# laboshinl/loam_velodyne

Hardware: AMD Instinct MI355X
Metric: sweeps/sec (64-ring, 1M-pt map): feature extraction + odometry + scan-to-map registration (higher is better)
Workload: dtype f32

## Files before the change

loam_velodyne_amd/csrc/dev_math.hpp:

```cpp
#pragma once
#include <hip/hip_runtime.h>
#include <cfloat>

namespace loamx {

struct Pose {
  float rx, ry, rz, tx, ty, tz;
  float srx, crx, sry, cry, srz, crz;
};

__host__ __device__ inline void pose_set_angles(Pose& p, float rx, float ry, float rz) {
  p.rx = rx; p.ry = ry; p.rz = rz;
  p.srx = (float)sin((double)rx); p.crx = (float)cos((double)rx);
  p.sry = (float)sin((double)ry); p.cry = (float)cos((double)ry);
  p.srz = (float)sin((double)rz); p.crz = (float)cos((double)rz);
}

__host__ __device__ inline void rot_x(float& y, float& z, float c, float s) {
  float y0 = y;
  y = c * y0 - s * z;
  z = s * y0 + c * z;
}
__host__ __device__ inline void rot_y(float& x, float& z, float c, float s) {
  float x0 = x;
// ... 183 lines not shown
#pragma unroll
      for (int r = k; r < M; r++) A[r][c] -= dot * v[r];
    }
    {
      float dot = 0.f;
#pragma unroll
      for (int r = k; r < M; r++) dot += v[r] * b[r];
      dot *= tau;
#pragma unroll
      for (int r = k; r < M; r++) b[r] -= dot * v[r];
    }
  }
  float y[N];
#pragma unroll
  for (int c = 0; c < N; c++) y[c] = 0.f;
#pragma unroll
  for (int k = N - 1; k >= 0; k--) {
    if (k < nonzero) {
      float s = b[k];
#pragma unroll
      for (int c = k + 1; c < N; c++)
        if (c < nonzero) s -= A[k][c] * y[c];
      y[k] = s / A[k][k];
    }
  }
#pragma unroll
  for (int c = 0; c < N; c++) x[c] = 0.f;
#pragma unroll
  for (int c = 0; c < N; c++)
#pragma unroll
    for (int j = 0; j < N; j++)
      if (c < nonzero && perm[c] == j) x[j] = y[c];
}

__device__ __forceinline__ void eig6_sym(const float* Ain, float* w, float* V, float* ws) {
  float* A = ws;
  float* Q = ws + 36;
  for (int r = 0; r < 6; r++)
    for (int c = 0; c <= r; c++) A[r * 6 + c] = A[c * 6 + r] = Ain[r * 6 + c];
  for (int r = 0; r < 6; r++)
    for (int c = 0; c < 6; c++) Q[r * 6 + c] = (r == c) ? 1.f : 0.f;
  for (int sweep = 0; sweep < 16; sweep++) {
    float off = 0.f, diag = 0.f;
    for (int r = 0; r < 6; r++) {
      diag += A[r * 6 + r] * A[r * 6 + r];
      for (int c = 0; c < r; c++) off += A[r * 6 + c] * A[r * 6 + c];
    }
    if (off <= 1e-20f * diag || off == 0.f) break;
    for (int p = 0; p < 5; p++)
      for (int q = p + 1; q < 6; q++) {
        float apq = A[p * 6 + q];
        if (apq == 0.f) continue;
        float theta = (A[q * 6 + q] - A[p * 6 + p]) / (2.f * apq);
        float t = (theta >= 0.f ? 1.f : -1.f) / (fabsf(theta) + sqrtf(theta * theta + 1.f));
        float c = 1.f / sqrtf(t * t + 1.f), s = t * c;
        for (int k = 0; k < 6; k++) {
          float akp = A[k * 6 + p], akq = A[k * 6 + q];
          A[k * 6 + p] = c * akp - s * akq;
          A[k * 6 + q] = s * akp + c * akq;
        }
        for (int k = 0; k < 6; k++) {
          float apk = A[p * 6 + k], aqk = A[q * 6 + k];
          A[p * 6 + k] = c * apk - s * aqk;
          A[q * 6 + k] = s * apk + c * aqk;
        }
        for (int k = 0; k < 6; k++) {
          float qkp = Q[k * 6 + p], qkq = Q[k * 6 + q];
          Q[k * 6 + p] = c * qkp - s * qkq;
          Q[k * 6 + q] = s * qkp + c * qkq;
        }
      }
  }
  int order[6];
#pragma unroll
  for (int k = 0; k < 6; k++) order[k] = k;
#pragma unroll
  for (int a_ = 1; a_ < 6; a_++) {
#pragma unroll
    for (int b_ = 5; b_ > 0; b_--) {
      if (b_ <= a_) {
        const float eb = A[order[b_] * 6 + order[b_]], ea = A[order[b_ - 1] * 6 + order[b_ - 1]];
        if (eb < ea) { int t = order[b_]; order[b_] = order[b_ - 1]; order[b_ - 1] = t; }
      }
    }
  }
  for (int k = 0; k < 6; k++) {
    w[k] = A[order[k] * 6 + order[k]];
    for (int r = 0; r < 6; r++) V[r * 6 + k] = Q[r * 6 + order[k]];
  }
}

__device__ __forceinline__ bool inverse6(const float* Ain, float* inv, float* ws) {
  float* A = ws;
  for (int r = 0; r < 6; r++)
    for (int c = 0; c < 6; c++) {
      A[r * 12 + c] = Ain[r * 6 + c];
      A[r * 12 + 6 + c] = (r == c) ? 1.f : 0.f;
    }
  for (int k = 0; k < 6; k++) {
    int piv = k;
    for (int r = k + 1; r < 6; r++)
      if (fabsf(A[r * 12 + k]) > fabsf(A[piv * 12 + k])) piv = r;
    if (A[piv * 12 + k] == 0.f) return false;
    if (piv != k)
      for (int c = 0; c < 12; c++) { float t = A[k * 12 + c]; A[k * 12 + c] = A[piv * 12 + c]; A[piv * 12 + c] = t; }
    float d = 1.f / A[k * 12 + k];
    for (int c = 0; c < 12; c++) A[k * 12 + c] *= d;
    for (int r = 0; r < 6; r++)
      if (r != k) {
        float f = A[r * 12 + k];
        if (f != 0.f)
          for (int c = 0; c < 12; c++) A[r * 12 + c] -= f * A[k * 12 + c];
      }
  }
  for (int r = 0; r < 6; r++)
    for (int c = 0; c < 6; c++) inv[r * 6 + c] = A[r * 12 + 6 + c];
  return true;
}

__device__ __forceinline__ bool certainly_not_degenerate(const float* AtA, float thr) {
  double L[6][6];
  const double shift = (double)thr * 1.001;
  double scale = 0.0;
#pragma unroll
  for (int i = 0; i < 6; i++) scale = fmax(scale, fabs((double)AtA[i * 6 + i]));
  const double tiny = 1e-6 * scale;
#pragma unroll
  for (int j = 0; j < 6; j++) {
    double dj = (double)AtA[j * 6 + j] - shift;
#pragma unroll
    for (int k = 0; k < 6; k++)
      if (k < j) dj -= L[j][k] * L[j][k];
    if (!(dj > tiny)) return false;
    const double lj = sqrt(dj);
    L[j][j] = lj;
#pragma unroll
    for (int i = 0; i < 6; i++)
      if (i > j) {
        double s = (double)AtA[i * 6 + j];
#pragma unroll
        for (int k = 0; k < 6; k++)
          if (k < j) s -= L[i][k] * L[j][k];
        L[i][j] = s / lj;
      }
  }
  return true;
}

__device__ __forceinline__ bool degeneracy_projector_full(const float* AtA, float thr, float* P, float* ws);
__device__ __forceinline__ bool degeneracy_projector(const float* AtA, float thr, float* P, float* ws) {
  if (certainly_not_degenerate(AtA, thr)) return false;
  return degeneracy_projector_full(AtA, thr, P, ws);
}
__device__ __forceinline__ bool degeneracy_projector_full(const float* AtA, float thr, float* P, float* ws) {
  float w[6];
  float* V = ws + 72;
  float* V2 = ws + 108;
  float* Vi = ws + 144;
  eig6_sym(AtA, w, V, ws);
  for (int k = 0; k < 36; k++) V2[k] = V[k];
  bool degenerate = false;
  {
    bool go = true;
#pragma unroll
    for (int i = 0; i < 6; i++) {
      if (go && w[i] < thr) {
        for (int j = 0; j < 6; j++) V2[i * 6 + j] = 0.f;
        degenerate = true;
      } else {
        go = false;
      }
    }
  }
  if (!inverse6(V, Vi, ws)) {
    for (int k = 0; k < 36; k++) P[k] = (k % 7 == 0) ? 1.f : 0.f;
    return degenerate;
  }
  for (int r = 0; r < 6; r++)
    for (int c = 0; c < 6; c++) {
      float s = 0.f;
      for (int k = 0; k < 6; k++) s += Vi[r * 6 + k] * V2[k * 6 + c];
      P[r * 6 + c] = s;
    }
  return degenerate;
}

__device__ __forceinline__ float lane_get(float x, int lane) { return __int_as_float(__builtin_amdgcn_readlane(__float_as_int(x), lane)); }

__device__ __forceinline__ float qr_solve6_lanes(const float* AtA, const float* AtB) {
  const int gl = (int)(threadIdx.x & 63);
  float a[6];
#pragma unroll
  for (int r = 0; r < 6; r++) a[r] = gl < 6 ? AtA[r * 6 + gl] : (gl == 6 ? AtB[r] : 0.f);
  int L[6] = {0, 1, 2, 3, 4, 5};
  bool pivoted = false;
  float s0 = 0.f;
#pragma unroll
  for (int r = 0; r < 6; r++) s0 += a[r] * a[r];
  const float nrm = gl < 6 ? sqrtf(s0) : 0.f;
  float maxnorm = lane_get(nrm, 0);
#pragma unroll
  for (int c = 1; c < 6; c++) {
    const float v = lane_get(nrm, c);
    maxnorm = v > maxnorm ? v : maxnorm;
  }
  const float thr_helper = (maxnorm * FLT_EPSILON) * (maxnorm * FLT_EPSILON) / 6.0f;
  int nonzero = 6;
#pragma unroll
  for (int k = 0; k < 6; k++) {
    float s = 0.f, tail = 0.f;
#pragma unroll
    for (int r = k; r < 6; r++) s += a[r] * a[r];
#pragma unroll
    for (int r = k + 1; r < 6; r++) tail += a[r] * a[r];
    const float c0 = a[k];
    float tau, beta, v[6];
    if (tail <= FLT_MIN) {
      tau = 0.f;
      beta = c0;
#pragma unroll
      for (int r = 0; r < 6; r++) v[r] = 0.f;
    } else {
      beta = sqrtf(c0 * c0 + tail);
      if (c0 >= 0.f) beta = -beta;
#pragma unroll
      for (int r = 0; r < 6; r++) v[r] = r > k ? a[r] / (c0 - beta) : 0.f;
      tau = (beta - c0) / beta;
    }
    v[k] = 1.f;
    int best = k;
    float bestn = lane_get(s, L[k]);
#pragma unroll
    for (int c = k + 1; c < 6; c++) {
      const float sc = lane_get(s, L[c]);
      if (sc > bestn) { bestn = sc; best = c; }
    }
    best = __builtin_amdgcn_readfirstlane(best);
    if (nonzero == 6 && bestn < thr_helper * float(6 - k)) nonzero = k;
    {
      int lb = L[k];
#pragma unroll
      for (int c = k + 1; c < 6; c++) lb = best == c ? L[c] : lb;
#pragma unroll
      for (int c = k + 1; c < 6; c++) L[c] = best == c ? L[k] : L[c];
      L[k] = __builtin_amdgcn_readfirstlane(lb);
    }
    const int pl = L[k];
    tau = lane_get(tau, pl);
    beta = lane_get(beta, pl);
#pragma unroll
    for (int r = k + 1; r < 6; r++) v[r] = lane_get(v[r], pl);
    if (gl == pl) {
      pivoted = true;
      a[k] = beta;
#pragma unroll
      for (int r = k + 1; r < 6; r++) a[r] = 0.f;
    } else if (gl <= 6 && !pivoted) {
      float dot = 0.f;
#pragma unroll
      for (int r = k; r < 6; r++) dot += v[r] * a[r];
      dot *= tau;
#pragma unroll
      for (int r = k; r < 6; r++) a[r] -= dot * v[r];
    }
  }
  float y = 0.f;
#pragma unroll
  for (int k = 5; k >= 0; k--) {
    float sacc = lane_get(a[k], 6);
#pragma unroll
    for (int c = k + 1; c < 6; c++) {
      const float term = lane_get(a[k] * y, L[c]);
      if (c < nonzero) sacc -= term;
    }
    const float diag = lane_get(a[k], L[k]);
    if (gl == L[k] && k < nonzero) y = sacc / diag;
  }
  return gl < 6 ? y : 0.f;
}
__device__ __forceinline__ void qr_solve6_coop(const float* AtA, const float* AtB, float* X) {
  const float y = qr_solve6_lanes(AtA, AtB);
  if ((threadIdx.x & 63) < 6) X[threadIdx.x & 63] = y;
}

__device__ __forceinline__ void xchg_store(double* p, double v) { __hip_atomic_store(p, v, __ATOMIC_RELAXED, __HIP_MEMORY_SCOPE_AGENT); }
__device__ __forceinline__ void xchg_stores_done() { asm volatile("s_waitcnt vmcnt(0)" ::: "memory"); }
__device__ __forceinline__ double xchg_load_nowait(const double* p) {
  double v;
  asm volatile("global_load_dwordx2 %0, %1, off sc1" : "=v"(v) : "v"(p) : "memory");
  return v;
}
typedef unsigned xrec_t __attribute__((ext_vector_type(4)));
__device__ __forceinline__ void xrec_store(xrec_t* p, double v, unsigned tag) {
  xrec_t r;
  r.x = tag; r.y = (unsigned)__double2loint(v); r.z = (unsigned)__double2hiint(v); r.w = tag;
  asm volatile("global_store_dwordx4 %0, %1, off sc1\n\ts_nop 1" ::"v"(p), "v"(r) : "memory");
}
__device__ __forceinline__ xrec_t xrec_load(const xrec_t* p) {
  xrec_t r;
  asm volatile("global_load_dwordx4 %0, %1, off sc1\n\ts_waitcnt vmcnt(0)" : "=v"(r) : "v"(p) : "memory");
  return r;
}
__device__ __forceinline__ double xrec_value(const xrec_t& r) { return __hiloint2double((int)r.z, (int)r.y); }
__device__ __forceinline__ void xchg_loads_done() { asm volatile("s_waitcnt vmcnt(0)" ::: "memory"); }
__device__ __forceinline__ void xchg_loaded(double& v) { asm volatile("" : "+v"(v)); }

}
```

loam_velodyne_amd/csrc/odometry.hip:

```cpp
#include "odometry.hpp"
#include "odom_schedule.hpp"
#include "pinned_copy.hpp"
#include <chrono>
#include <cstring>
#include <type_traits>

namespace loamx {

constexpr int OD_THREADS = 256;
constexpr int OD_TR_STRIDE = OD_THREADS + 2;
constexpr int OD_PART_STRIDE = 2 * (2 * 16 * LX_NSUM) + 16;
[[maybe_unused]] constexpr int OD_PART_TS = 2 * (2 * 16 * LX_NSUM);

__device__ inline void sincos_f(float a, float& s, float& c) { sincosf(a, &s, &c); }

__device__ inline void transform_to_start(const float* T, float scan_period, const float4 pi, float& x, float& y, float& z) {
  const float s = (1.f / scan_period) * (pi.w - (float)(int)pi.w);
  x = pi.x - s * T[3];
  y = pi.y - s * T[4];
  z = pi.z - s * T[5];
  float sx, cx, sy, cy, sz, cz;
  sincos_f(-s * T[0], sx, cx);
  sincos_f(-s * T[1], sy, cy);
  sincos_f(-s * T[2], sz, cz);
// ... 124 lines not shown
template <bool LOAD_FIRST, class F>
__device__ inline void block27_scan(const Block27& B, const float4* __restrict__ sorted, int lane, Block27First& first, F&& visit) {
  for (uint32_t c0 = (uint32_t)lane; c0 < B.total; c0 += 4 * 64) {
    const bool first_trip = c0 == (uint32_t)lane;
    uint32_t pos[4];
    float4 p[4];
#pragma unroll
    for (int u = 0; u < 4; u++) {
      const uint32_t cc = c0 + 64u * u;
      uint32_t o = B.O[8];
#pragma unroll
      for (int k = 7; k >= 0; k--) o = cc < B.E[k] ? B.O[k] : o;
      pos[u] = cc < B.total ? cc + o : B.O[0];
    }
    if (LOAD_FIRST || !first_trip) {
#pragma unroll
      for (int u = 0; u < 4; u++) p[u] = sorted[pos[u]];
      if (LOAD_FIRST && first_trip) {
#pragma unroll
        for (int u = 0; u < OD_BLK_CACHE; u++) first.p[u] = p[u];
      }
    } else {
#pragma unroll
      for (int u = OD_BLK_CACHE; u < 4; u++) p[u] = sorted[pos[u]];
#pragma unroll
      for (int u = 0; u < OD_BLK_CACHE; u++) p[u] = first.p[u];
    }
#pragma unroll
    for (int u = 0; u < 4; u++) visit(p[u], (c0 + 64u * u) < B.total);
  }
}
__device__ inline int nn1_block(const GridDesc& g, const Block27& B, const float4* __restrict__ sorted, const uint32_t* __restrict__ cell_start,
                                float qx, float qy, float qz, int lane, uint32_t& w_out, Block27First& first) {
  float lbest = 25.0f;
  uint32_t lw = 0xffffffffu;
  block27_scan<true>(B, sorted, lane, first, [&](const float4& p, bool valid) {
    const float dx = qx - p.x, dy2 = qy - p.y, dz2 = qz - p.z;
    const float d2 = dx * dx + dy2 * dy2 + dz2 * dz2;
    const uint32_t w = __float_as_uint(p.w);
    if (valid && (d2 < lbest || (d2 == lbest && lw != 0xffffffffu && (w & OD_IDX_MASK) < (lw & OD_IDX_MASK)))) { lbest = d2; lw = w; }
  });
  float d = lbest;
  int j = lw == 0xffffffffu ? -1 : (int)(lw & OD_IDX_MASK), o_ = lw == 0xffffffffu ? 0x7fffffff : (int)(lw & OD_IDX_MASK);
  int ring = (int)(lw >> 24);
  {
#pragma unroll
    for (int off = 32; off > 0; off >>= 1) {
      const float od = __shfl_xor(d, off, 64);
      const int oj = __shfl_xor(j, off, 64), oo = __shfl_xor(o_, off, 64), orr = __shfl_xor(ring, off, 64);
      if (od < d || (od == d && oo < o_)) { d = od; j = oj; o_ = oo; ring = orr; }
    }
  }
  const float h = 1.0f / g.inv_h;
  if (j >= 0 && d < 25.0f && d <= h * h) { w_out = ((uint32_t)ring << 24) | (uint32_t)j; return j; }
  const int id = nn1_shells(g, sorted, cell_start, qx, qy, qz, lane, 2, (j >= 0 && d < 25.0f) ? d : 25.0f, (j >= 0 && d < 25.0f) ? j : -1);
  w_out = id == j ? (((uint32_t)ring << 24) | (uint32_t)j) : (0xff000000u | (uint32_t)(id < 0 ? 0 : id));
  return id;
}

constexpr int OD_RF_N = 320;
#ifdef LOAMX_PROF_CORR
__device__ unsigned long long g_corr_ts[3][16];
#define OC_TS(k) do { if (blockIdx.y == 0 && lane == 0 && ts_slot >= 0) g_corr_ts[ts_slot][k] = wall_clock64(); } while (0)
#else
#define OC_TS(k) do { } while (0)
#endif
__global__ __launch_bounds__(256) OD_CORR_ATTR void k_odom_corr_grid(OdomProblem* __restrict__ probs, OdomParams P, uint32_t* __restrict__ patch_dst, uint4 patch) {
  if (patch_dst && blockIdx.x == 0 && blockIdx.y == 0 && threadIdx.x == 0) { patch_dst[0] = patch.x; patch_dst[1] = patch.y; patch_dst[2] = patch.z; }
  OdomProblem& pb = probs[blockIdx.y];
  if (pb.done) return;
  const int lane = threadIdx.x & 63, wid = threadIdx.x >> 6;
  const int nSharp = (int)pb.n_sharp, nFlat = (int)pb.n_flat;
  int f;
  {
    const int x = (int)(blockIdx.x % 8), j = (int)(blockIdx.x / 8);
    const int sS = (int)((long long)x * nSharp / 8), nS = (int)((long long)(x + 1) * nSharp / 8) - sS;
    const int sF = (int)((long long)x * nFlat / 8), nF = (int)((long long)(x + 1) * nFlat / 8) - sF;
    const int fl = 4 * j + wid;
    if (fl >= nS + nF) return;
    f = fl < nS ? sS + fl : nSharp + sF + (fl - nS);
  }
#ifdef LOAMX_PROF_CORR
  const int ts_slot = f == nSharp / 2 ? 0 : f == nSharp + nFlat / 2 ? 1 : f == nSharp + nFlat - 1 ? 2 : -1;
#endif
  OC_TS(0);
  float T[6];
#pragma unroll
  for (int k = 0; k < 6; k++) T[k] = pb.transform[k];
  const bool corner = f < nSharp;
  const float4 pi = corner ? pb.sharp[f] : pb.flat[f - nSharp];
  const uint32_t* __restrict__ tbl = corner ? pb.rf_corner : pb.rf_surf;
  const int e0 = max((int)pi.w - 8, 0);
  uint32_t tv = 0u, unordered_epoch = 0u;
  if (tbl) {
    if (e0 + lane < OD_RF_N - 1) tv = tbl[e0 + lane];
    unordered_epoch = tbl[OD_RF_N - 1];
  }
  float x, y, z;
  transform_to_start(T, P.scan_period, pi, x, y, z);
  const GridDescB gd = corner ? *pb.lc_desc : *pb.ls_desc;
  const float4* __restrict__ sorted = pb.sorted;
  const uint32_t* __restrict__ cell_start = pb.cell_table + gd.cell_base;
  OC_TS(1);
  Block27 B;
  block27_build(gd.g, cell_start, x, y, z, lane, B);
  OC_TS(2);
  uint32_t wbest = 0u;
  Block27First first;
  const int closest = nn1_block(gd.g, B, sorted, cell_start, x, y, z, lane, wbest, first);
  OC_TS(3);
  if (closest < 0) {
    if (lane == 0) { pb.ind[5 * f] = -1; pb.ind[5 * f + 1] = -1; pb.ind[5 * f + 2] = -1; }
    return;
  }
  const float4* last = corner ? pb.last_corner : pb.last_surf;
  const int nLast = corner ? (int)pb.n_last_corner : (int)pb.n_last_surf;
  const int nCur = corner ? nSharp : nFlat;
  const int bound = nCur < nLast ? nCur : nLast;
  const int cscan = (wbest >> 24) != 255u ? (int)(wbest >> 24) : (int)last[closest].w;
  float d2 = 25.f, d3 = 25.f;
  int j2 = -1, j3 = -1, o2 = 0x7fffffff, o3 = 0x7fffffff;
  auto better = [](float d, int order, float dbest, int obest) { return d < dbest || (d == dbest && obest != 0x7fffffff && order < obest); };

  bool via_block = false;
  if (tbl && unordered_epoch != pb.rf_epoch && cscan < 255 && B.total > 0u) {
    const unsigned long long valid = __ballot(e0 + lane < OD_RF_N - 1 && (tv >> 24) == pb.rf_epoch);
    auto first_from = [&](int ring) -> int {
      const int k = ring - e0;
      if (k >= 64) return nLast;
      const unsigned long long m = k <= 0 ? valid : (valid >> k) << k;
      if (!m) return nLast;
      const int w = (int)((uint32_t)__shfl((int)tv, __builtin_ctzll(m), 64) & OD_IDX_MASK);
      return w < nLast ? w : nLast;
    };
    if (cscan - 2 >= e0 || e0 == 0) {
      const int wlo = min(first_from(cscan - 2), closest);
      const int whi = closest + 1 < bound ? max(min(bound, first_from(cscan + 3)), closest + 1) : closest + 1;
      const unsigned walk = (unsigned)(closest - wlo) + (unsigned)(whi - (closest + 1));
      via_block = walk > B.total + 128u;
    }
  }
  OC_TS(4);
  if (via_block) {
    block27_scan<false>(B, sorted, lane, first, [&](const float4& p, bool ok) {
      const uint32_t w = __float_as_uint(p.w);
      const int j = (int)(w & OD_IDX_MASK), ring = (int)(w >> 24);
      const float d = sqd(p, x, y, z);
      if (ok && j > closest && j < bound && ring <= cscan + 2) {
        const int order = j - (closest + 1);
        if (corner) {
          if (ring > cscan && better(d, order, d2, o2)) { d2 = d; j2 = j; o2 = order; }
        } else {
          if (ring <= cscan) { if (better(d, order, d2, o2)) { d2 = d; j2 = j; o2 = order; } }
          else { if (better(d, order, d3, o3)) { d3 = d; j3 = j; o3 = order; } }
        }
      } else if (ok && j < closest && ring >= cscan - 2) {
        const int order = 0x40000000 + (closest - 1 - j);
        if (corner) {
          if (ring < cscan && better(d, order, d2, o2)) { d2 = d; j2 = j; o2 = order; }
        } else {
          if (ring >= cscan) { if (better(d, order, d2, o2)) { d2 = d; j2 = j; o2 = order; } }
          else { if (better(d, order, d3, o3)) { d3 = d; j3 = j; o3 = order; } }
        }
      }
    });
    wave_argmin(d2, j2, o2);
    if (!corner) wave_argmin(d3, j3, o3);
    const float h = 1.0f / gd.g.inv_h, h2 = h * h;
    via_block = d2 < h2 && (corner || d3 < h2);
    if (!via_block) { d2 = d3 = 25.f; j2 = j3 = -1; o2 = o3 = 0x7fffffff; }
  }
  OC_TS(5);
  if (!via_block) {
    int baseF = closest + 1, baseB = closest - 1;
    bool stopF = baseF >= bound, stopB = baseB < 0;
    while (!stopF || !stopB) {
      float4 qf[4], qb[4];
      if (!stopF) {
#pragma unroll
        for (int u = 0; u < 4; u++) {
          const int j = baseF + 64 * u + lane;
          qf[u] = j < bound ? last[j] : make_float4(0.f, 0.f, 0.f, 0.f);
        }
      }
      if (!stopB) {
#pragma unroll
        for (int u = 0; u < 4; u++) {
          const int j = baseB - 64 * u - lane;
          qb[u] = j >= 0 ? last[j] : make_float4(0.f, 0.f, 0.f, 0.f);
        }
      }
      if (!stopF) {
        bool stop = false;
#pragma unroll
        for (int u = 0; u < 4; u++) {
          if (stop) continue;
          const int j = baseF + 64 * u + lane;
          const bool in = j < bound;
          const int ring = (int)qf[u].w;
          const bool brk = in && ((double)ring > (double)cscan + 2.5);
          const unsigned long long mb = __ballot(brk);
          const int fb = mb ? __builtin_ctzll(mb) : 64;
          if (in && lane < fb) {
            const float d = sqd(qf[u], x, y, z);
            const int order = j - (closest + 1);
            if (corner) {
              if (ring > cscan && better(d, order, d2, o2)) { d2 = d; j2 = j; o2 = order; }
            } else {
              if (ring <= cscan) { if (better(d, order, d2, o2)) { d2 = d; j2 = j; o2 = order; } }
              else { if (better(d, order, d3, o3)) { d3 = d; j3 = j; o3 = order; } }
            }
          }
          if (mb) stop = true;
        }
        baseF += 256;
        stopF = stop || baseF >= bound;
      }
      if (!stopB) {
        bool stop = false;
#pragma unroll
        for (int u = 0; u < 4; u++) {
          if (stop) continue;
          const int j = baseB - 64 * u - lane;
          const bool in = j >= 0;
          const int ring = (int)qb[u].w;
          const bool brk = in && ((double)ring < (double)cscan - 2.5);
          const unsigned long long mb = __ballot(brk);
          const int fb = mb ? __builtin_ctzll(mb) : 64;
          if (in && lane < fb) {
            const float d = sqd(qb[u], x, y, z);
            const int order = 0x40000000 + (closest - 1 - j);
            if (corner) {
              if (ring < cscan && better(d, order, d2, o2)) { d2 = d; j2 = j; o2 = order; }
            } else {
              if (ring >= cscan) { if (better(d, order, d2, o2)) { d2 = d; j2 = j; o2 = order; } }
              else { if (better(d, order, d3, o3)) { d3 = d; j3 = j; o3 = order; } }
            }
          }
          if (mb) stop = true;
        }
        baseB -= 256;
        stopB = stop || baseB < 0;
      }
    }
    wave_argmin(d2, j2, o2);
    if (!corner) wave_argmin(d3, j3, o3);
  }
  OC_TS(6);
  if (lane == 0) {
    pb.ind[5 * f] = closest;
    pb.ind[5 * f + 1] = j2;
    pb.ind[5 * f + 2] = corner ? -1 : j3;
  }
#ifdef LOAMX_PROF_CORR
  if (blockIdx.y == 0 && lane == 0 && ts_slot >= 0) {
    g_corr_ts[ts_slot][7] = wall_clock64();
    g_corr_ts[ts_slot][8] = (unsigned long long)B.total; g_corr_ts[ts_slot][9] = (unsigned long long)via_block;
    g_corr_ts[ts_slot][10] = (unsigned long long)closest; g_corr_ts[ts_slot][11] = (unsigned long long)cscan;
  }
#endif
}

#ifdef LOAMX_PROF_LM
#define LM_TS(k) do { if (blockIdx.x == 0 && blockIdx.y == 0 && tid == 0 && iter == it_begin + 1) pb.part[OD_PART_TS + (k)] = (double)wall_clock64(); } while (0)
#else
#define LM_TS(k) do { } while (0)
#endif
#ifndef OD_LM_WAVES
#define OD_LM_WAVES 3
#endif
#ifndef OD_LM_WAVES_MIN
#define OD_LM_WAVES_MIN 3
#endif
#define OD_LM_ATTR __attribute__((amdgpu_waves_per_eu(OD_LM_WAVES_MIN, OD_LM_WAVES)))
#pragma clang diagnostic push
#pragma clang diagnostic ignored "-Wpass-failed"
template <int OD_FPT>
__global__ __launch_bounds__(OD_THREADS) OD_LM_ATTR void k_odom_lm(OdomProblem* __restrict__ probs, OdomParams P, int iter0, int n_iters) {
  OdomProblem& pb = probs[blockIdx.y];
  if (pb.done) return;
  const unsigned NB = gridDim.x;
  const int tid = threadIdx.x;
  const int nSharp = (int)pb.n_sharp, nFlat = (int)pb.n_flat, nFeat = nSharp + nFlat;
  __shared__ float T[6];
  __shared__ float trig[6];
  __shared__ double red[8][LX_NSUM];
  using TrT = typename std::conditional<OD_FPT == 1, float, double>::type;
  __shared__ TrT tr[LX_NSUM * OD_TR_STRIDE];
  __shared__ int sh_done, sh_degen, sh_abort;
  __shared__ float matP[36];
  __shared__ float ws[216];
  __shared__ double parts[16 * LX_NSUM];
  __shared__ float AtA[36], AtB[6];
  if (tid < 6) {
    T[tid] = pb.transform[tid];
    const double ang = (double)pb.transform[tid >> 1];
    trig[tid] = (float)((tid & 1) ? cos(ang) : sin(ang));
  }
  const unsigned xtag = pb.xchg_epoch << 8;
  if (tid == 0) { sh_done = 0; sh_abort = 0; sh_degen = pb.stats.degenerate; }
  if (tid < 36) matP[tid] = pb.matP[tid];
  __syncthreads();

  float4 fpo[OD_FPT], ft1[OD_FPT], ft2[OD_FPT], ft3[OD_FPT];
  bool fvalid[OD_FPT], fcorner[OD_FPT];
#pragma unroll
  for (int u = 0; u < OD_FPT; u++) {
    const int f = (u * (int)NB + (int)blockIdx.x) * OD_THREADS + tid;
    fvalid[u] = false;
    fcorner[u] = f < nSharp;
    fpo[u] = ft1[u] = ft2[u] = ft3[u] = make_float4(0.f, 0.f, 0.f, 0.f);
    if (f < nFeat) {
      const int i1 = pb.ind[5 * f], i2 = pb.ind[5 * f + 1], i3 = pb.ind[5 * f + 2];
      if (fcorner[u] ? (i2 >= 0) : (i2 >= 0 && i3 >= 0)) {
        fvalid[u] = true;
        fpo[u] = fcorner[u] ? pb.sharp[f] : pb.flat[f - nSharp];
        const float4* last = fcorner[u] ? pb.last_corner : pb.last_surf;
        ft1[u] = last[i1];
        ft2[u] = last[i2];
        if (!fcorner[u]) ft3[u] = last[i3];
      }
    }
  }

  const int it_begin = iter0, it_end = iter0 + n_iters;
  for (int iter = it_begin; iter < it_end; iter++) {
    LM_TS(0);
    LM_TS(1);
    double v[OD_FPT == 1 ? 1 : LX_NSUM];
    float a1[6] = {0.f, 0.f, 0.f, 0.f, 0.f, 0.f}, bb1 = 0.f;
    bool sel1 = false;
#pragma unroll
    for (int k = 0; k < (OD_FPT == 1 ? 1 : LX_NSUM); k++) v[k] = 0.0;
#pragma unroll
    for (int u = 0; u < OD_FPT; u++) {
      if (!fvalid[u]) continue;
      const bool corner = fcorner[u];
      const float4 po = fpo[u];
      float cx = 0.f, cy = 0.f, cz = 0.f, ci = 0.f;
      bool sel = false;
      {
        float x0, y0, z0;
        transform_to_start(T, P.scan_period, po, x0, y0, z0);
        if (corner) {
          const float4 t1 = ft1[u], t2 = ft2[u];
          const float x1 = t1.x, y1 = t1.y, z1 = t1.z, x2 = t2.x, y2 = t2.y, z2 = t2.z;
          const float a012 = sqrtf(((x0 - x1) * (y0 - y2) - (x0 - x2) * (y0 - y1)) * ((x0 - x1) * (y0 - y2) - (x0 - x2) * (y0 - y1)) +
                                   ((x0 - x1) * (z0 - z2) - (x0 - x2) * (z0 - z1)) * ((x0 - x1) * (z0 - z2) - (x0 - x2) * (z0 - z1)) +
                                   ((y0 - y1) * (z0 - z2) - (y0 - y2) * (z0 - z1)) * ((y0 - y1) * (z0 - z2) - (y0 - y2) * (z0 - z1)));
          const float l12 = sqrtf((x1 - x2) * (x1 - x2) + (y1 - y2) * (y1 - y2) + (z1 - z2) * (z1 - z2));
          const float la = ((y1 - y2) * ((x0 - x1) * (y0 - y2) - (x0 - x2) * (y0 - y1)) +
                            (z1 - z2) * ((x0 - x1) * (z0 - z2) - (x0 - x2) * (z0 - z1))) / a012 / l12;
          const float lb = -((x1 - x2) * ((x0 - x1) * (y0 - y2) - (x0 - x2) * (y0 - y1)) -
                             (z1 - z2) * ((y0 - y1) * (z0 - z2) - (y0 - y2) * (z0 - z1))) / a012 / l12;
          const float lc = -((x1 - x2) * ((x0 - x1) * (z0 - z2) - (x0 - x2) * (z0 - z1)) +
                             (y1 - y2) * ((y0 - y1) * (z0 - z2) - (y0 - y2) * (z0 - z1))) / a012 / l12;
          const float ld2 = a012 / l12;
          float s = 1;
          if (iter >= 5) s = 1 - 1.8f * fabsf(ld2);
          cx = s * la; cy = s * lb; cz = s * lc; ci = s * ld2;
          sel = ((double)s > 0.1) && (ld2 != 0);
        } else {
          const float4 t1 = ft1[u], t2 = ft2[u], t3 = ft3[u];
          float pa = (t2.y - t1.y) * (t3.z - t1.z) - (t3.y - t1.y) * (t2.z - t1.z);
          float pbb = (t2.z - t1.z) * (t3.x - t1.x) - (t3.z - t1.z) * (t2.x - t1.x);
          float pc = (t2.x - t1.x) * (t3.y - t1.y) - (t3.x - t1.x) * (t2.y - t1.y);
          float pd = -(pa * t1.x + pbb * t1.y + pc * t1.z);
          const float ps = sqrtf(pa * pa + pbb * pbb + pc * pc);
          pa /= ps; pbb /= ps; pc /= ps; pd /= ps;
          const float pd2 = pa * x0 + pbb * y0 + pc * z0 + pd;
          float s = 1;
          if (iter >= 5) s = 1 - 1.8f * fabsf(pd2) / sqrtf(sqrtf(x0 * x0 + y0 * y0 + z0 * z0));
          cx = s * pa; cy = s * pbb; cz = s * pc; ci = s * pd2;
          sel = ((double)s > 0.1) && (pd2 != 0);
        }
      }
      if (sel) {
        const float srx = trig[0], crx = trig[1], sry = trig[2], cry = trig[3], srz = trig[4], crz = trig[5];
        const float tx = T[3], ty = T[4], tz = T[5];
        const float px = po.x, py = po.y, pz = po.z;
        float a[6];
        a[0] = (-crx * sry * srz * px + crx * crz * sry * py + srx * sry * pz + tx * crx * sry * srz - ty * crx * crz * sry - tz * srx * sry) * cx +
               (srx * srz * px - crz * srx * py + crx * pz + ty * crz * srx - tz * crx - tx * srx * srz) * cy +
               (crx * cry * srz * px - crx * cry * crz * py - cry * srx * pz + tz * cry * srx + ty * crx * cry * crz - tx * crx * cry * srz) * cz;
        a[1] = ((-crz * sry - cry * srx * srz) * px + (cry * crz * srx - sry * srz) * py - crx * cry * pz + tx * (crz * sry + cry * srx * srz) +
                ty * (sry * srz - cry * crz * srx) + tz * crx * cry) * cx +
               ((cry * crz - srx * sry * srz) * px + (cry * srz + crz * srx * sry) * py - crx * sry * pz + tz * crx * sry -
                ty * (cry * srz + crz * srx * sry) - tx * (cry * crz - srx * sry * srz)) * cz;
        a[2] = ((-cry * srz - crz * srx * sry) * px + (cry * crz - srx * sry * srz) * py + tx * (cry * srz + crz * srx * sry) -
                ty * (cry * crz - srx * sry * srz)) * cx +
               (-crx * crz * px - crx * srz * py + ty * crx * srz + tx * crx * crz) * cy +
               ((cry * crz * srx - sry * srz) * px + (crz * sry + cry * srx * srz) * py + tx * (sry * srz - cry * crz * srx) -
                ty * (crz * sry + cry * srx * srz)) * cz;
        a[3] = -(cry * crz - srx * sry * srz) * cx + crx * srz * cy - (crz * sry + cry * srx * srz) * cz;
        a[4] = -(cry * srz + crz * srx * sry) * cx - crx * crz * cy - (sry * srz - cry * crz * srx) * cz;
        a[5] = crx * sry * cx - srx * cy - crx * cry * cz;
        const float bb = (float)(-0.05 * (double)ci);
        if (OD_FPT == 1) {
#pragma unroll
          for (int i = 0; i < 6; i++) a1[i] = a[i];
          bb1 = bb;
          sel1 = true;
        } else {
          int k = 0;
#pragma unroll
          for (int i = 0; i < 6; i++)
#pragma unroll
            for (int j = i; j < 6; j++) v[k++] += (double)(a[i] * a[j]);
#pragma unroll
          for (int i = 0; i < 6; i++) v[k++] += (double)(a[i] * bb);
          v[k] += 1.0;
        }
      }
    }
    LM_TS(2);
    if (OD_FPT == 1) {
      int k = 0;
#pragma unroll
      for (int i = 0; i < 6; i++)
#pragma unroll
        for (int j = i; j < 6; j++) tr[(k++) * OD_TR_STRIDE + tid] = (TrT)(a1[i] * a1[j]);
#pragma unroll
      for (int i = 0; i < 6; i++) tr[(k++) * OD_TR_STRIDE + tid] = (TrT)(a1[i] * bb1);
      tr[k * OD_TR_STRIDE + tid] = (TrT)(sel1 ? 1.f : 0.f);
    } else {
#pragma unroll
      for (int t = 0; t < LX_NSUM; t++) tr[t * OD_TR_STRIDE + tid] = (TrT)v[OD_FPT == 1 ? 0 : t];
    }
    __syncthreads();
    if (tid < 8 * LX_NSUM) {
      const int c = tid % LX_NSUM, g = tid / LX_NSUM;
      const TrT* col = tr + c * OD_TR_STRIDE + g;
      double x = 0.0;
#pragma unroll 8
      for (int j = 0; j < OD_THREADS / 8; j++) x += (double)col[8 * j];
      red[g][c] = x;
    }
    __syncthreads();
    LM_TS(3);
    double xs = 0.0;
    if (tid < LX_NSUM) {
#pragma unroll
      for (int w = 0; w < 8; w++) xs += red[w][tid];
      if (NB > 1) {
        xrec_store(reinterpret_cast<xrec_t*>(pb.part) + (((unsigned)iter & 1u) * 16u + blockIdx.x) * LX_NSUM + tid, xs, xtag | (unsigned)(iter + 1));
      }
    }
    if (NB > 1) {
      LM_TS(4);
      {
        const unsigned want = xtag | (unsigned)(iter + 1);
        const xrec_t* rec = reinterpret_cast<const xrec_t*>(pb.part) + ((unsigned)iter & 1u) * 16u * LX_NSUM;
        const unsigned long long t_in = wall_clock64();
        for (unsigned e = tid; e < NB * LX_NSUM; e += OD_THREADS) {
          unsigned spins = 0;
          xrec_t r = xrec_load(rec + e);
          while (r.x != want || r.w != want) {
            __builtin_amdgcn_s_sleep(1);
            if ((++spins & 1023u) == 0u && wall_clock64() - t_in > 200000000ull) { sh_abort = 1; break; }
            r = xrec_load(rec + e);
          }
          parts[e] = xrec_value(r);
        }
      }
      __syncthreads();
      if (sh_abort) {
        if (tid == 0) {
          pb.done = 1;
          if (pb.err_word) __hip_atomic_store(pb.err_word, 1u, __ATOMIC_RELAXED, __HIP_MEMORY_SCOPE_SYSTEM);
          if (pb.host_mirror) pb.host_mirror->done = -1;
        }
        return;
      }
      LM_TS(5);
    }
    if (tid < 64) {
      if (NB > 1 && tid < LX_NSUM) {
        xs = 0.0;
        for (unsigned b = 0; b < NB; b++) xs += parts[b * LX_NSUM + tid];
      }
      if (tid < 21) {
        int i = 0, rem = tid;
        while (rem >= 6 - i) { rem -= 6 - i; i++; }
        const int j = i + rem;
        AtA[i * 6 + j] = AtA[j * 6 + i] = (float)xs;
      } else if (tid < 27) {
        AtB[tid - 21] = (float)xs;
      }
      const int sel = (int)__hiloint2double(__builtin_amdgcn_readlane(__double2hiint(xs), 27), __builtin_amdgcn_readlane(__double2loint(xs), 27));
      __builtin_amdgcn_fence(__ATOMIC_SEQ_CST, "wavefront");
      LM_TS(7);
      float xl = 0.f;
      int done_now = 0;
      if (sel >= 10) {
        xl = qr_solve6_lanes(AtA, AtB);
        LM_TS(8);
        if (iter == 0) {
          if (tid == 0) sh_degen = degeneracy_projector(AtA, 10.f, matP, ws) ? 1 : 0;
          __builtin_amdgcn_fence(__ATOMIC_SEQ_CST, "wavefront");
          if (blockIdx.x == 0 && tid < 36) pb.matP[tid] = matP[tid];
        }
        const int degen = sh_degen;
        if (degen) {
          const int r = tid < 6 ? tid : 5;
          float acc = 0.f;
#pragma unroll
          for (int c = 0; c < 6; c++) acc += matP[r * 6 + c] * lane_get(xl, c);
          xl = acc;
        }
        float x6[6];
#pragma unroll
        for (int k = 0; k < 6; k++) x6[k] = lane_get(xl, k);
        const float d0 = (float)(x6[0] * 180.0 / M_PI), d1 = (float)(x6[1] * 180.0 / M_PI), d2 = (float)(x6[2] * 180.0 / M_PI);
        const float deltaR = (float)sqrt((double)d0 * d0 + (double)d1 * d1 + (double)d2 * d2);
        const float t0 = x6[3] * 100, t1 = x6[4] * 100, t2 = x6[5] * 100;
        const float deltaT = (float)sqrt((double)t0 * t0 + (double)t1 * t1 + (double)t2 * t2);
        done_now = (deltaR < P.delta_r_abort && deltaT < P.delta_t_abort) ? 1 : 0;
      }
      float tl = T[tid < 6 ? tid : 5];
      if (sel >= 10) {
        float nv = tl + xl;
        if (!isfinite(nv)) nv = 0.f;
        tl = nv;
      }
      const float a0 = lane_get(tl, 0), a1 = lane_get(tl, 1), a2 = lane_get(tl, 2);
      const double ang = (double)((tid >> 1) == 0 ? a0 : ((tid >> 1) == 1 ? a1 : a2));
      const float tg = (float)((tid & 1) ? cos(ang) : sin(ang));
      if (tid < 6) { T[tid] = tl; trig[tid] = tg; }
      if (tid == 0 && done_now) sh_done = 1;
      if (blockIdx.x == 0) {
        const bool final_now = done_now || iter == it_end - 1;
        if (tid < 6) pb.transform[tid] = tl;
        if (tid == 0) {
          pb.stats.iterations = iter + 1;
          pb.stats.sel = sel;
          if (iter == 0 && sel >= 10) pb.stats.degenerate = sh_degen;
          if (done_now) pb.done = 1;
        }
        if (final_now) {
          ToEndParams& Pe = *pb.te_out;
          if (tid < 6) {
            Pe.T[tid] = tl;
            if (tid & 1) Pe.cT[tid >> 1] = tg; else Pe.sT[tid >> 1] = tg;
          }
          if (pb.host_mirror) {
            OdomProblem* hm = pb.host_mirror;
            if (tid < 6) hm->transform[tid] = tl;
            if (tid == 0) {
              OdomStats stt;
              stt.iterations = iter + 1; stt.sel = sel; stt.frame = pb.stats.frame; stt.degenerate = sh_degen;
              hm->stats = stt;
              hm->done = done_now;
            }
          }
        }
      }
      LM_TS(9);
    }
    __syncthreads();
    if (sh_done) break;
  }
}

#pragma clang diagnostic pop

__device__ inline float4 to_end_point(float4 p, const ToEndParams& P) {
  const float s = (1.f / P.scan_period) * (p.w - (float)(int)p.w);
  float x = p.x - s * P.T[3], y = p.y - s * P.T[4], z = p.z - s * P.T[5];
  float sx, cx, sy, cy, sz, cz;
  sincos_f(-s * P.T[0], sx, cx);
  sincos_f(-s * P.T[1], sy, cy);
  sincos_f(-s * P.T[2], sz, cz);
  rot_z(x, y, cz, sz); rot_x(y, z, cx, sx); rot_y(x, z, cy, sy);
  rot_y(x, z, P.cT[1], P.sT[1]); rot_x(y, z, P.cT[0], P.sT[0]); rot_z(x, y, P.cT[2], P.sT[2]);
  x += P.T[3] - P.shift[0];
  y += P.T[4] - P.shift[1];
  z += P.T[5] - P.shift[2];
  rot_z(x, y, P.c_start[2], P.s_start[2]); rot_x(y, z, P.c_start[0], P.s_start[0]); rot_y(x, z, P.c_start[1], P.s_start[1]);
  rot_y(x, z, P.c_end[1], -P.s_end[1]); rot_x(y, z, P.c_end[0], -P.s_end[0]); rot_z(x, y, P.c_end[2], -P.s_end[2]);
  return make_float4(x, y, z, (float)(int)p.w);
}
__global__ __launch_bounds__(256) void k_transform_to_end_copy(float4* __restrict__ dst, const float4* __restrict__ src, uint32_t n, ToEndParams P) {
  const uint32_t i = blockIdx.x * blockDim.x + threadIdx.x;
  if (i >= n) return;
  dst[i] = to_end_point(src[i], P);
}
__global__ __launch_bounds__(256) void k_transform_to_end(float4* __restrict__ pts, uint32_t n, ToEndParams P) {
  const uint32_t i = blockIdx.x * blockDim.x + threadIdx.x;
  if (i >= n) return;
  pts[i] = to_end_point(pts[i], P);
}
__global__ void k_te_patch(const OdomProblem* __restrict__ probs, uint32_t na, ToEndParams* __restrict__ te) {
  const uint32_t a = blockIdx.x * blockDim.x + threadIdx.x;
  if (a >= na) return;
  const OdomProblem& pb = probs[a];
  ToEndParams& P = te[pb.stream_id];
  for (int k = 0; k < 6; k++) P.T[k] = pb.transform[k];
  for (int k = 0; k < 3; k++) {
    P.sT[k] = (float)sin((double)pb.transform[k]);
    P.cT[k] = (float)cos((double)pb.transform[k]);
  }
}

__global__ __launch_bounds__(256) void k_transform_to_end_batch(float4* __restrict__ pts, uint32_t n, const uint32_t* __restrict__ off,
                                                                uint32_t K, uint32_t ns, const ToEndParams* __restrict__ params,
                                                                const float4* __restrict__ src_c, const float4* __restrict__ src_s,
                                                                uint32_t n_corner_all, uint32_t* __restrict__ bounds,
                                                                uint32_t* __restrict__ ring_first, uint32_t rf_epoch) {
  const uint32_t i = blockIdx.x * blockDim.x + threadIdx.x;
  const bool active = i < n;
  uint32_t lo = 0;
  float4 q = make_float4(0.f, 0.f, 0.f, 0.f);
  if (active) {
    uint32_t hi = K;
    while (hi - lo > 1) {
      const uint32_t mid = (lo + hi) >> 1;
      if (off[mid] <= i) lo = mid; else hi = mid;
    }
    const ToEndParams P = params[lo % ns];
    if (src_c) {
      const float4 p = i < n_corner_all ? src_c[i] : src_s[i - n_corner_all];
      q = P.enabled ? to_end_point(p, P) : p;
      pts[i] = q;
    } else {
      q = pts[i];
      if (P.enabled) { q = to_end_point(q, P); pts[i] = q; }
    }
  }
  if (ring_first) {
    const int ring = (int)q.w;
    int prev = __shfl_up(ring, 1, 64);
    const uint32_t plo = (uint32_t)__shfl_up((int)lo, 1, 64);
    const bool first_in_cloud = active && i == off[lo];
    if (active && !first_in_cloud && (threadIdx.x & 63) == 0) {
      const uint32_t ip = i - 1;
      prev = (int)(src_c ? (ip < n_corner_all ? src_c[ip] : src_s[ip - n_corner_all]) : pts[ip]).w;
    } else if (active && plo != lo) {
      prev = -1;
    }
    if (active && ring >= 0 && ring < OD_RF_N - 1 && (first_in_cloud || prev != ring))
      ring_first[(size_t)lo * OD_RF_N + ring] = (rf_epoch << 24) | ((i - off[lo]) & OD_IDX_MASK);
    if (active && (ring < 0 || ring >= 255 || (i - off[lo]) > OD_IDX_MASK || (!first_in_cloud && prev > ring)))
      ring_first[(size_t)lo * OD_RF_N + OD_RF_N - 1] = rf_epoch;
  }
  if (bounds) cloud_bounds_update(bounds, active, lo, q.x, q.y, q.z);
}

__global__ __launch_bounds__(256) void k_to_end_gather(float4* __restrict__ dst, uint32_t n, const uint32_t* __restrict__ off, uint32_t K,
                                                       const float4* const* __restrict__ src, const uint32_t* __restrict__ sid,
                                                       const ToEndParams* __restrict__ params) {
  const uint32_t i = blockIdx.x * blockDim.x + threadIdx.x;
  if (i >= n) return;
  uint32_t lo = 0, hi = K;
  while (hi - lo > 1) {
    const uint32_t mid = (lo + hi) >> 1;
    if (off[mid] <= i) lo = mid; else hi = mid;
  }
  dst[i] = to_end_point(src[lo][i - off[lo]], params[sid[lo]]);
}

OdometryBatch::OdometryBatch(int device, uint32_t n_streams, hipStream_t shared_stream) : device_(device) {
  select_device(device);
  LX_REQUIRE(n_streams >= 1 && n_streams <= 1024, "n_streams must be in [1, 1024]");
  if (shared_stream) {
    st_ = shared_stream;
  } else {
    st_ = create_stream(env_priority("LOAMX_PRIO_ODOM", +1), 0, 0);
    own_stream_ = true;
  }
  for (uint32_t s = 0; s < n_streams; s++) streams_.push_back(new OdomStream());
  index_.cell_size = 2.1f;
  if (const char* e = diag_env("LOAMX_ODOM_CELL")) { const float v = (float)atof(e); if (v >= 0.25f && v <= 16.f) index_.cell_size = v; }
  index_.pack_ring = true;
  index_.init(st_);
  h_mirror_.reserve(n_streams);
  h_err_.reserve(16);
  rf_.reserve((size_t)2 * n_streams * OD_RF_N);
  LX_HIP(hipMemsetAsync(rf_.p, 0, sizeof(uint32_t) * 2 * n_streams * OD_RF_N, st_));
  memset(h_err_.p, 0, 16 * sizeof(uint32_t));
  part_.reserve((size_t)n_streams * OD_PART_STRIDE);
  LX_HIP(hipMemset(part_.p, 0, sizeof(double) * part_.cap));
  {
    auto up256 = [](size_t b) { return (b + 255) & ~(size_t)255; };
    const size_t o_te = up256(sizeof(OdomProblem) * n_streams), o_off = o_te + up256(sizeof(ToEndParams) * n_streams);
    up_bytes_ = o_off + up256(sizeof(uint32_t) * (2 * (size_t)n_streams + 2));
    up_dev_.reserve(up_bytes_);
    up_host_.reserve(up_bytes_);
    memset(up_host_.p, 0, up_bytes_);
    prob_.p = (OdomProblem*)up_dev_.p; h_prob_.p = (OdomProblem*)up_host_.p;
    te_.p = (ToEndParams*)(up_dev_.p + o_te); h_te_.p = (ToEndParams*)(up_host_.p + o_te);
    d_cur_off_.p = (uint32_t*)(up_dev_.p + o_off); h_off_pin_.p = (uint32_t*)(up_host_.p + o_off);
  }
  h_cur_off_.assign(2 * n_streams + 1, 0);
  h_last_off_.assign(2 * n_streams + 1, 0);
}

OdometryBatch::~OdometryBatch() {
  if (ev_tail_) (void)hipEventDestroy(ev_tail_);
  if (ev_up_) (void)hipEventDestroy(ev_up_);
  if (ev_pose_) (void)hipEventDestroy(ev_pose_);
  for (auto* p : streams_) delete p;
  for (auto& c : lt_) for (auto& e : c.ev) if (e) (void)hipEventDestroy(e);
  if (own_stream_ && st_) (void)hipStreamDestroy(st_);
}

void OdometryBatch::lt_resolve_() {
  for (auto& c : lt_) {
    if (!c.pending || !c.pairs) continue;
    if (hipEventQuery(c.ev[3 * (c.pairs - 1) + 2]) != hipSuccess) { (void)hipGetLastError(); continue; }
    for (int k = 0; k < c.pairs; k++) {
      float a = 0.f, b = 0.f;
      if (hipEventElapsedTime(&a, c.ev[3 * k], c.ev[3 * k + 1]) != hipSuccess || hipEventElapsedTime(&b, c.ev[3 * k + 1], c.ev[3 * k + 2]) != hipSuccess) { (void)hipGetLastError(); continue; }
      if (c.iters[k] > 0) {
        lt_tot_.corr_ms += a; lt_tot_.corr_launches++; lt_tot_.corr_features += c.feats[k];
        lt_tot_.lm_ms += b; lt_tot_.lm_launches++; lt_tot_.lm_iterations += (uint64_t)c.iters[k]; lt_tot_.lm_bytes += c.bytes[k];
      } else {
        lt_tot_.corr_noop_ms += a; lt_tot_.corr_noop_launches++;
        lt_tot_.lm_noop_ms += b; lt_tot_.lm_noop_launches++;
      }
    }
    c.pending = false;
  }
}
OdometryBatch::LaunchTotals OdometryBatch::launch_totals() {
  std::lock_guard<std::mutex> lk(lt_mu_);
  lt_resolve_();
  return lt_tot_;
}

void odom_set_imu(OdomStream& S, const float* t);
ToEndParams odom_to_end_params(const OdomStream& S, float scan_period, bool enabled);
void odom_integrate_pose(OdomStream& S);

void OdometryBatch::update_imu(uint32_t s, const float* t) { odom_set_imu(*streams_[s], t); }

ToEndParams OdometryBatch::to_end_params(uint32_t s, bool enabled) const { return odom_to_end_params(*streams_[s], params.scan_period, enabled); }

void OdometryBatch::to_end_device(uint32_t s, float4* pts, uint32_t n) {
  if (!n) return;
  hipLaunchKernelGGL(k_transform_to_end, dim3((n + 255) / 256), dim3(256), 0, st_, pts, n, to_end_params(s, true));
}

void odom_integrate_pose(OdomStream& S) {
  HAngle rx, ry, rz;
  accumulate_rotation(S.transform_sum.rot_x, S.transform_sum.rot_y, S.transform_sum.rot_z, -S.transform.rot_x,
                      HAngle((float)(-S.transform.rot_y.r * 1.05)), -S.transform.rot_z, rx, ry, rz);
  HVec3 v{S.transform.pos.x - S.imu_shift.x, S.transform.pos.y - S.imu_shift.y, (float)(S.transform.pos.z * 1.05 - S.imu_shift.z)};
  h_rot_zxy(v, rz, rx, ry);
  HVec3 trans{S.transform_sum.pos.x - v.x, S.transform_sum.pos.y - v.y, S.transform_sum.pos.z - v.z};
  plugin_imu_rotation(rx, ry, rz, S.imu_pitch_start, S.imu_yaw_start, S.imu_roll_start, S.imu_pitch_end, S.imu_yaw_end,
                      S.imu_roll_end, rx, ry, rz);
  S.transform_sum.rot_x = rx; S.transform_sum.rot_y = ry; S.transform_sum.rot_z = rz;
  S.transform_sum.pos = trans;
}
void odom_set_imu(OdomStream& S, const float* t) {
  S.imu_pitch_start = HAngle(t[0]); S.imu_yaw_start = HAngle(t[1]); S.imu_roll_start = HAngle(t[2]);
  S.imu_pitch_end = HAngle(t[3]); S.imu_yaw_end = HAngle(t[4]); S.imu_roll_end = HAngle(t[5]);
  S.imu_shift = {t[6], t[7], t[8]};
  S.imu_velo = {t[9], t[10], t[11]};
}
ToEndParams odom_to_end_params(const OdomStream& S, float scan_period, bool enabled) {
  ToEndParams P;
  S.transform.get(P.T);
  const HAngle* ta[3] = {&S.transform.rot_x, &S.transform.rot_y, &S.transform.rot_z};
  const HAngle* sa[3] = {&S.imu_pitch_start, &S.imu_yaw_start, &S.imu_roll_start};
// ... 475 lines not shown
```

Baseline: 16250.

## Precompute per-feature line/plane constants and batch cross-block exchange loads in one wavefront

Each feature's plane coefficients (surface) and line length (corner) are now computed once before the LM iteration loop and kept in registers, so later iterations no longer recompute them. The cross-block partial-sum exchange now uses only the first 64 threads. They issue up to eight dwordx4 loads back to back with a single wait, then spin only on records that were not yet ready. This is meant to cut per-iteration latency on the grid-wide reduction, the serial bottleneck of the iterative solver. It holds 7 floats per feature slot in registers and assumes NB*LX_NSUM fits in 512 records (8 x 64).

```diff
diff --git a/loam_velodyne_amd/csrc/dev_math.hpp b/loam_velodyne_amd/csrc/dev_math.hpp
--- a/loam_velodyne_amd/csrc/dev_math.hpp
+++ b/loam_velodyne_amd/csrc/dev_math.hpp
@@ -509,6 +509,12 @@
   return r;
 }
 __device__ __forceinline__ double xrec_value(const xrec_t& r) { return __hiloint2double((int)r.z, (int)r.y); }
+__device__ __forceinline__ xrec_t xrec_load_nowait(const xrec_t* p) {
+  xrec_t r;
+  asm volatile("global_load_dwordx4 %0, %1, off sc1" : "=v"(r) : "v"(p) : "memory");
+  return r;
+}
+__device__ __forceinline__ void xrec_loaded(xrec_t& r) { asm volatile("" : "+v"(r)); }
 __device__ __forceinline__ void xchg_loads_done() { asm volatile("s_waitcnt vmcnt(0)" ::: "memory"); }
 __device__ __forceinline__ void xchg_loaded(double& v) { asm volatile("" : "+v"(v)); }
 
diff --git a/loam_velodyne_amd/csrc/odometry.hip b/loam_velodyne_amd/csrc/odometry.hip
--- a/loam_velodyne_amd/csrc/odometry.hip
+++ b/loam_velodyne_amd/csrc/odometry.hip
@@ -450,23 +450,38 @@
   if (tid < 36) matP[tid] = pb.matP[tid];
   __syncthreads();
 
-  float4 fpo[OD_FPT], ft1[OD_FPT], ft2[OD_FPT], ft3[OD_FPT];
+  float4 fpo[OD_FPT];
+  float fk[OD_FPT][7];
   bool fvalid[OD_FPT], fcorner[OD_FPT];
 #pragma unroll
   for (int u = 0; u < OD_FPT; u++) {
     const int f = (u * (int)NB + (int)blockIdx.x) * OD_THREADS + tid;
     fvalid[u] = false;
     fcorner[u] = f < nSharp;
-    fpo[u] = ft1[u] = ft2[u] = ft3[u] = make_float4(0.f, 0.f, 0.f, 0.f);
+    fpo[u] = make_float4(0.f, 0.f, 0.f, 0.f);
+#pragma unroll
+    for (int k = 0; k < 7; k++) fk[u][k] = 0.f;
     if (f < nFeat) {
       const int i1 = pb.ind[5 * f], i2 = pb.ind[5 * f + 1], i3 = pb.ind[5 * f + 2];
       if (fcorner[u] ? (i2 >= 0) : (i2 >= 0 && i3 >= 0)) {
         fvalid[u] = true;
         fpo[u] = fcorner[u] ? pb.sharp[f] : pb.flat[f - nSharp];
         const float4* last = fcorner[u] ? pb.last_corner : pb.last_surf;
-        ft1[u] = last[i1];
-        ft2[u] = last[i2];
-        if (!fcorner[u]) ft3[u] = last[i3];
+        const float4 t1 = last[i1], t2 = last[i2];
+        if (fcorner[u]) {
+          const float x1 = t1.x, y1 = t1.y, z1 = t1.z, x2 = t2.x, y2 = t2.y, z2 = t2.z;
+          const float l12 = sqrtf((x1 - x2) * (x1 - x2) + (y1 - y2) * (y1 - y2) + (z1 - z2) * (z1 - z2));
+          fk[u][0] = x1; fk[u][1] = y1; fk[u][2] = z1; fk[u][3] = x2; fk[u][4] = y2; fk[u][5] = z2; fk[u][6] = l12;
+        } else {
+          const float4 t3 = last[i3];
+          float pa = (t2.y - t1.y) * (t3.z - t1.z) - (t3.y - t1.y) * (t2.z - t1.z);
+          float pbb = (t2.z - t1.z) * (t3.x - t1.x) - (t3.z - t1.z) * (t2.x - t1.x);
+          float pc = (t2.x - t1.x) * (t3.y - t1.y) - (t3.x - t1.x) * (t2.y - t1.y);
+          float pd = -(pa * t1.x + pbb * t1.y + pc * t1.z);
+          const float ps = sqrtf(pa * pa + pbb * pbb + pc * pc);
+          pa /= ps; pbb /= ps; pc /= ps; pd /= ps;
+          fk[u][0] = pa; fk[u][1] = pbb; fk[u][2] = pc; fk[u][3] = pd;
+        }
       }
     }
   }
@@ -491,12 +506,10 @@
         float x0, y0, z0;
         transform_to_start(T, P.scan_period, po, x0, y0, z0);
         if (corner) {
-          const float4 t1 = ft1[u], t2 = ft2[u];
-          const float x1 = t1.x, y1 = t1.y, z1 = t1.z, x2 = t2.x, y2 = t2.y, z2 = t2.z;
+          const float x1 = fk[u][0], y1 = fk[u][1], z1 = fk[u][2], x2 = fk[u][3], y2 = fk[u][4], z2 = fk[u][5], l12 = fk[u][6];
           const float a012 = sqrtf(((x0 - x1) * (y0 - y2) - (x0 - x2) * (y0 - y1)) * ((x0 - x1) * (y0 - y2) - (x0 - x2) * (y0 - y1)) +
                                    ((x0 - x1) * (z0 - z2) - (x0 - x2) * (z0 - z1)) * ((x0 - x1) * (z0 - z2) - (x0 - x2) * (z0 - z1)) +
                                    ((y0 - y1) * (z0 - z2) - (y0 - y2) * (z0 - z1)) * ((y0 - y1) * (z0 - z2) - (y0 - y2) * (z0 - z1)));
-          const float l12 = sqrtf((x1 - x2) * (x1 - x2) + (y1 - y2) * (y1 - y2) + (z1 - z2) * (z1 - z2));
           const float la = ((y1 - y2) * ((x0 - x1) * (y0 - y2) - (x0 - x2) * (y0 - y1)) +
                             (z1 - z2) * ((x0 - x1) * (z0 - z2) - (x0 - x2) * (z0 - z1))) / a012 / l12;
           const float lb = -((x1 - x2) * ((x0 - x1) * (y0 - y2) - (x0 - x2) * (y0 - y1)) -
@@ -509,13 +522,7 @@
           cx = s * la; cy = s * lb; cz = s * lc; ci = s * ld2;
           sel = ((double)s > 0.1) && (ld2 != 0);
         } else {
-          const float4 t1 = ft1[u], t2 = ft2[u], t3 = ft3[u];
-          float pa = (t2.y - t1.y) * (t3.z - t1.z) - (t3.y - t1.y) * (t2.z - t1.z);
-          float pbb = (t2.z - t1.z) * (t3.x - t1.x) - (t3.z - t1.z) * (t2.x - t1.x);
-          float pc = (t2.x - t1.x) * (t3.y - t1.y) - (t3.x - t1.x) * (t2.y - t1.y);
-          float pd = -(pa * t1.x + pbb * t1.y + pc * t1.z);
-          const float ps = sqrtf(pa * pa + pbb * pbb + pc * pc);
-          pa /= ps; pbb /= ps; pc /= ps; pd /= ps;
+          const float pa = fk[u][0], pbb = fk[u][1], pc = fk[u][2], pd = fk[u][3];
           const float pd2 = pa * x0 + pbb * y0 + pc * z0 + pd;
           float s = 1;
           if (iter >= 5) s = 1 - 1.8f * fabsf(pd2) / sqrtf(sqrtf(x0 * x0 + y0 * y0 + z0 * z0));
@@ -596,19 +603,40 @@
     }
     if (NB > 1) {
       LM_TS(4);
-      {
+      if (tid < 64) {
         const unsigned want = xtag | (unsigned)(iter + 1);
         const xrec_t* rec = reinterpret_cast<const xrec_t*>(pb.part) + ((unsigned)iter & 1u) * 16u * LX_NSUM;
         const unsigned long long t_in = wall_clock64();
-        for (unsigned e = tid; e < NB * LX_NSUM; e += OD_THREADS) {
-          unsigned spins = 0;
-          xrec_t r = xrec_load(rec + e);
-          while (r.x != want || r.w != want) {
-            __builtin_amdgcn_s_sleep(1);
-            if ((++spins & 1023u) == 0u && wall_clock64() - t_in > 200000000ull) { sh_abort = 1; break; }
-            r = xrec_load(rec + e);
+        const unsigned nrec = NB * LX_NSUM;
+        unsigned pend = 0u;
+        unsigned lane = (unsigned)tid;
+        asm volatile("" : "+v"(lane));
+#pragma unroll
+        for (int u0 = 0; u0 < 8; u0 += 4) {
+          if (64u * u0 >= nrec) break;
+          xrec_t r[4];
+#pragma unroll
+          for (int u = 0; u < 4; u++) r[u] = xrec_load_nowait(rec + min(64u * (u0 + u) + lane, nrec - 1u));
+          xchg_loads_done();
+#pragma unroll
+          for (int u = 0; u < 4; u++) {
+            xrec_loaded(r[u]);
+            const unsigned e = 64u * (u0 + u) + lane;
+            if (e < nrec) {
+              if (r[u].x == want && r[u].w == want) parts[e] = xrec_value(r[u]);
+              else pend |= 1u << (u0 + u);
+            }
           }
-          parts[e] = xrec_value(r);
+        }
+        unsigned spins = 0;
+        while (pend) {
+          __builtin_amdgcn_s_sleep(1);
+          if ((++spins & 1023u) == 0u && wall_clock64() - t_in > 200000000ull) { sh_abort = 1; break; }
+          for (unsigned u = 0; 64u * u < nrec; u++)
+            if (pend & (1u << u)) {
+              const xrec_t q = xrec_load(rec + 64u * u + lane);
+              if (q.x == want && q.w == want) { parts[64u * u + lane] = xrec_value(q); pend &= ~(1u << u); }
+            }
         }
       }
       __syncthreads();
```

Result: no change. 16140, median of 2 (-0.7%).
